# zd87pl/ai-crypto-trader

Hardware: AMD Instinct MI355X
Metric: backtested_1m_candles_per_sec_ga_pop_eval (higher is better)
Workload: dtype fp32; 1 GPU; model=ga_backtest_evolution, global_batch=1024, seq_len=1000000, parallelism=dp1, symbols=64, pop_per_gpu=1024, fitness_segments=64

## Files before the change

ai_crypto_trader_amd/ops/hip/backtest.hip:

```cpp

#include "bt_position.hpp"

namespace {

struct BtState {
    VoteState v;
    BtPosition pos;

    __device__ void load(const float* __restrict__ pr, float initial_equity)
    {
        v.load(pr);
        pos.load(pr, initial_equity);
    }

    __device__ void step(int t, float close, float high, float low,
                         float change, float2 ms, float4 sv)
    {
#pragma clang fp contract(off)
        const int net =
            v.count(t, close, v.recur(t, close, change), ms, sv);
        pos.step(t, net, v.entry_v, v.exit_v, close, high, low);
    }
};

#define BT_BBSUB 32
static_assert(BT_TILE % BT_BBSUB == 0, "sub-tiles must tile the tile");
static_assert(BT_BLOCK % BT_MAXWIN == 0 && BT_BBSUB <= BT_BLOCK &&
                  (BT_MAXWIN & (BT_MAXWIN - 1)) == 0,
              "a lane converts slots of one window only");
static_assert(BT_MAXWIN <= BT_WARMUP, "early-window entries are unused");

__device__ inline float4 bt_pack_sums(double a, double b)
{
    return make_float4(__int_as_float(__double2loint(a)),
                       __int_as_float(__double2hiint(a)),
                       __int_as_float(__double2loint(b)),
                       __int_as_float(__double2hiint(b)));
}

__device__ inline double bt_unpack_sum(float lo, float hi)
{
    return __hiloint2double(__float_as_int(hi), __float_as_int(lo));
}

template <bool HAS_RESNAP>
__global__ void __launch_bounds__(BT_BLOCK, 5) backtest_kernel(
    const float* __restrict__ candles,
    const float* __restrict__ pop,
    float* __restrict__ metrics,
    int nsym, int T, int P, int chunks_per_sym, float initial_equity)
{
#pragma clang fp contract(off)
    __shared__ float chist[BT_SPAN];
    __shared__ double csq[BT_SPAN];
    __shared__ float hl[BT_SPAN][2];
    __shared__ float4 sh_vote[BT_TILE];
    __shared__ float4 bbtab[BT_BBSUB * BT_MAXWIN];
    __shared__ double sh_sum[BT_MAXWIN], sh_sum2[BT_MAXWIN];
    __shared__ double sh_invw[BT_MAXWIN];

    int sym, chunk;
    bt_block_map(blockIdx.x, nsym, chunks_per_sym, sym, chunk);
    const int tid = threadIdx.x;
    const int p = chunk * BT_BLOCK + tid;
    const bool act = p < P;

    BtState st;
    st.load(pop + (long)(act ? p : 0) * BT_NPARAM, initial_equity);
    const float4* my_bb = bbtab + (st.v.bb_w - 2);

    const int scan_w = tid + 2;
    const bool is_scan = scan_w <= BT_MAXWIN;
    if (tid < BT_MAXWIN) {
        BollState b;
        b.init(scan_w);
        sh_sum[tid] = b.sum;
        sh_sum2[tid] = b.sum2;
        sh_invw[tid] = b.inv_w;
    }
    if (tid < BT_BBSUB)
        bbtab[tid * BT_MAXWIN + BT_MAXWIN - 1] =
            make_float4(0.0f, 0.0f, 0.0f, 0.0f);

    float prev_close = 0.f;
    const float4* sym_candles =
        reinterpret_cast<const float4*>(candles + (long)sym * T * 4);

    for (int t0 = 0; t0 < T; t0 += BT_TILE) {
        bt_stage_tile(sym_candles, t0, T, chist, hl, csq);
        const int tend = min(BT_TILE, T - t0);
        const bool resnap_tile = HAS_RESNAP && (t0 > 0) &&
                                 ((t0 & (BT_RESNAP - 1)) == 0);
        if (resnap_tile && is_scan) {
            BollState b;
            b.resnap(scan_w, &chist[BT_HALO]);
            sh_sum[tid] = b.sum;
            sh_sum2[tid] = b.sum2;
        }
        bt_shared_votes(t0, tend, chist, hl, sh_vote);
        for (int s0 = 0; s0 < tend; s0 += BT_BBSUB) {
            const int send = min(s0 + BT_BBSUB, tend);
            if (s0 > 0) __syncthreads();
            if (is_scan) {
                BollState b;
                b.sum = sh_sum[tid];
                b.sum2 = sh_sum2[tid];
#pragma unroll 4
                for (int tt = s0; tt < send; ++tt) {
                    const int i = tt + BT_HALO;
                    if (!(resnap_tile && tt == 0))
                        b.advance(chist[i], chist[i - scan_w], csq[i],
                                  csq[i - scan_w]);
                    bbtab[(tt - s0) * BT_MAXWIN + tid] =
                        bt_pack_sums(b.sum, b.sum2);
                }
                sh_sum[tid] = b.sum;
                sh_sum2[tid] = b.sum2;
            }
            __syncthreads();
            {
                BollState b;
                b.inv_w = sh_invw[tid & (BT_MAXWIN - 1)];
                for (int e = tid; e < (send - s0) * BT_MAXWIN;
                     e += BT_BLOCK) {
                    const float4 v = bbtab[e];
                    b.sum = bt_unpack_sum(v.x, v.y);
                    b.sum2 = bt_unpack_sum(v.z, v.w);
                    const float2 ms = b.stats<false>(0, 0);
                    bbtab[e].x = ms.x;
                    bbtab[e].y = ms.y;
                }
            }
            __syncthreads();
            for (int tt = s0; tt < send; ++tt) {
                const int t = t0 + tt;
                const float close = chist[tt + BT_HALO];
                const float high = hl[tt + BT_HALO][0];
                const float low = hl[tt + BT_HALO][1];
                const float change = (t == 0) ? 0.0f : close - prev_close;
                const float4 sv = sh_vote[tt];
                const float4* e = &my_bb[(tt - s0) * BT_MAXWIN];
                st.step(t, close, high, low, change,
                        make_float2(e->x, e->y), sv);
                prev_close = close;
            }
        }
    }

    if (act)
        st.pos.acc.finalize(metrics + ((long)p * nsym + sym) * BT_NMETRIC, T);
}

}

extern "C" void launch_backtest(const float* candles, const float* pop,
                                float* metrics, int nsym, int T, int P,
                                float initial_equity, hipStream_t stream) {
    const int chunks = (P + BT_BLOCK - 1) / BT_BLOCK;
    auto k = T > BT_RESNAP ? backtest_kernel<true> : backtest_kernel<false>;
    hipLaunchKernelGGL(k, dim3(nsym * chunks), dim3(BT_BLOCK), 0, stream,
                       candles, pop, metrics, nsym, T, P, chunks,
                       initial_equity);
}
```

ai_crypto_trader_amd/ops/hip/bt_common.hpp:

```cpp
#pragma once

#include "common.hpp"

#define BT_BLOCK 256
#define BT_TILE 256
#define BT_NMETRIC 10
#define BT_FEE 0.001f
#define BT_EPS 1e-9f
#define BT_ANNUALIZE 0x1.6a7dccp+9f

__device__ inline void bt_write_metrics(
    float* __restrict__ out, int T, float equity, float n_trades,
    float wins, float gross_p, float gross_l, float max_dd, float sum_ret,
    float sum_ret2)
{
#pragma clang fp contract(off)
    float n = (float)max(T, 1);
    float mean_r = sum_ret / n;
    float var_r = fmaxf(sum_ret2 / n - mean_r * mean_r, 0.0f);
    float sharpe = mean_r / fmaxf(sqrtf(var_r), BT_EPS) * BT_ANNUALIZE;
    if (!(n_trades > 0.0f)) sharpe = 0.0f;
    float win_rate = wins / fmaxf(n_trades, 1.0f);
    float fitness = (n_trades > 0.0f)
                        ? sharpe + win_rate - 2.0f * max_dd
                        : -1.0f;
    out[0] = equity; out[1] = n_trades; out[2] = wins;
    out[3] = gross_p; out[4] = gross_l; out[5] = max_dd;
    out[6] = sum_ret; out[7] = sum_ret2;
    out[8] = sharpe; out[9] = fitness;
}

struct BtAccum {
    float equity, max_eq, max_dd;
    float n_trades, wins, gross_p, gross_l;
    float sum_ret, sum_ret2;

    __device__ void init(float initial_equity)
    {
        equity = initial_equity; max_eq = initial_equity; max_dd = 0.f;
        n_trades = wins = gross_p = gross_l = 0.f;
        sum_ret = sum_ret2 = 0.f;
    }

    __device__ void trade(float pnl)
    {
        n_trades += 1.0f;
        wins += (pnl > 0.0f) ? 1.0f : 0.0f;
        gross_p += fmaxf(pnl, 0.0f);
        gross_l += fmaxf(-pnl, 0.0f);
    }

    __device__ void mark(float new_eq)
    {
#pragma clang fp contract(off)
        float r = new_eq / equity - 1.0f;
        sum_ret += r;
        sum_ret2 += r * r;
        equity = new_eq;
        max_eq = fmaxf(max_eq, equity);
        max_dd = fmaxf(max_dd, (max_eq - equity) / max_eq);
    }

    __device__ void finalize(float* __restrict__ out, int T) const
    {
        bt_write_metrics(out, T, equity, n_trades, wins, gross_p, gross_l,
                         max_dd, sum_ret, sum_ret2);
    }
};

__device__ inline void bt_block_map(int bid, int nsym, int chunks_per_sym,
                                    int& sym, int& chunk)
{
    int nblocks = nsym * chunks_per_sym;
    if ((nsym & 7) == 0 && (nblocks & 7) == 0) {
        int xcd = bid & 7, j = bid >> 3;
        sym = xcd + 8 * (j / chunks_per_sym);
        chunk = j % chunks_per_sym;
    } else {
        sym = bid / chunks_per_sym;
        chunk = bid % chunks_per_sym;
    }
}
```

ai_crypto_trader_amd/ops/hip/bt_position.hpp:

```cpp
#pragma once

#include "bt_vote.hpp"

#define BT_EV_NONE 0
#define BT_EV_STOP 1
#define BT_EV_TP 2
#define BT_EV_SIGNAL 3
#define BT_EV_ENTRY (-1)

struct BtEvent {
    int kind;
    float price;
    float pnl;
};

struct BtPosition {
    float size_pct, sl_pct, tp_pct, trail_pct, trail_act;
    float cash, units;
    bool in_pos;
    float entry_cost, entry_price;
    float stop, tp, peak;
    BtAccum acc;

    __device__ void load(const float* __restrict__ pr, float initial_equity)
    {
        size_pct = pr[12]; sl_pct = pr[13]; tp_pct = pr[14];
        trail_pct = pr[15]; trail_act = pr[16];
        cash = initial_equity; units = 0.f;
        in_pos = false;
        entry_cost = entry_price = stop = tp = peak = 0.f;
        acc.init(initial_equity);
    }

    __device__ BtEvent step(int t, int net, int entry_v, int exit_v,
                            float close, float high, float low)
    {
#pragma clang fp contract(off)
        BtEvent ev = {BT_EV_NONE, 0.0f, 0.0f};
        if (in_pos) {
            peak = fmaxf(peak, high);
            bool trail_on = (trail_pct > 0.0f) &&
                            (peak >= entry_price * (1.0f + trail_act));
            if (trail_on)
                stop = fmaxf(stop, peak * (1.0f - trail_pct));
            bool hit_sl = low <= stop;
            bool hit_tp = !hit_sl && high >= tp;
            bool hit_sig = !hit_sl && !hit_tp && net <= -exit_v;
            if (hit_sl || hit_tp || hit_sig) {
                float exit_price = hit_sl ? stop : (hit_tp ? tp : close);
                float proceeds = units * exit_price * (1.0f - BT_FEE);
                cash += proceeds;
                acc.trade(proceeds - entry_cost);
                ev.kind = hit_sl ? BT_EV_STOP
                                 : (hit_tp ? BT_EV_TP : BT_EV_SIGNAL);
                ev.price = exit_price;
                ev.pnl = proceeds - entry_cost;
                units = 0.0f;
                in_pos = false;
            }
        } else if (t >= BT_WARMUP && net >= entry_v) {
            float cost = fminf(size_pct * acc.equity, cash);
            units = cost * (1.0f - BT_FEE) / close;
            cash -= cost;
            entry_cost = cost;
            entry_price = close;
            stop = close * (1.0f - sl_pct);
            tp = close * (1.0f + tp_pct);
            peak = close;
            in_pos = true;
            ev.kind = BT_EV_ENTRY;
        }

        if (units != 0.0f || cash != acc.equity)
            acc.mark(cash + units * close);
        return ev;
    }
};
```

ai_crypto_trader_amd/ops/hip/bt_vote.hpp:

```cpp
#pragma once

#include "bt_common.hpp"

#define BT_NPARAM 19
#define BT_MAXWIN 32
#define BT_HALO 64
#define BT_SPAN (BT_TILE + BT_HALO)
#define BT_WARMUP 128
#define BT_RESNAP 16384
#define BT_NSTATE 18

struct BollState {
    double sum, sum2, inv_w;

    __device__ void init(int w)
    {
        sum = sum2 = 0.0;
        inv_w = 1.0 / (double)w;
    }

    __device__ void resnap(int w, const float* __restrict__ hist)
    {
#pragma clang fp contract(off)
        double s = 0.0, s2 = 0.0;
        for (int j = BT_MAXWIN - 1; j >= 0; --j) {
            if (j < w) {
                double c = (double)hist[-j];
                s += c;
                s2 += c * c;
            }
        }
        sum = s;
        sum2 = s2;
    }

    __device__ void advance(float close, float oldc, double csq_new,
                            double csq_old)
    {
#pragma clang fp contract(off)
        double old = (double)oldc;
        double c64 = (double)close;
        sum += c64 - old;
        sum2 += csq_new - csq_old;
    }

    template <bool EARLY = true>
    __device__ float2 stats(int t, int w) const
    {
#pragma clang fp contract(off)
        double inv_cnt = inv_w;
        if (EARLY && t < BT_MAXWIN && t + 1 < w)
            inv_cnt = 1.0 / (t + 1.0);
        double mean64 = sum * inv_cnt;
        double var64 = fmax(sum2 * inv_cnt - mean64 * mean64, 0.0);
        return make_float2((float)mean64, sqrtf((float)var64));
    }
};

struct VoteState {
    float inv_rsi_p, rsi_os, rsi_ob;
    float a_f, a_s, a_sig;
    int bb_w;
    float bb_k, bb_bth, bb_sth;
    int entry_v, exit_v;
    float stoch_os, stoch_ob, will_os, will_ob;

    float ema_f, ema_s, sig;
    float avg_gain, avg_loss;
    BollState bb;

    __device__ void load(const float* __restrict__ pr)
    {
        inv_rsi_p = 1.0f / fmaxf(floorf(pr[0]), 1.0f);
        rsi_os = pr[1]; rsi_ob = pr[2];
        a_f = 2.0f / (pr[3] + 1.0f);
        a_s = 2.0f / (pr[4] + 1.0f);
        a_sig = 2.0f / (pr[5] + 1.0f);
        bb_w = min(max((int)pr[6], 2), BT_MAXWIN);
        bb_k = pr[7]; bb_bth = pr[8]; bb_sth = pr[9];
        entry_v = (int)pr[10]; exit_v = (int)pr[11];
        stoch_os = pr[17]; stoch_ob = pr[18];
        will_os = stoch_os - 100.0f;
        will_ob = stoch_ob - 100.0f;
        ema_f = ema_s = sig = 0.f;
        avg_gain = avg_loss = 0.f;
        bb.init(bb_w);
    }

    __device__ void resnap(const float* __restrict__ hist)
    {
        bb.resnap(bb_w, hist);
    }

    __device__ void warm_step(float close, float change)
    {
#pragma clang fp contract(off)
        ema_f += a_f * (close - ema_f);
        ema_s += a_s * (close - ema_s);
        float macd = ema_f - ema_s;
        sig += a_sig * (macd - sig);
        float gain = fmaxf(change, 0.0f);
        float loss = fmaxf(-change, 0.0f);
        avg_gain += (gain - avg_gain) * inv_rsi_p;
        avg_loss += (loss - avg_loss) * inv_rsi_p;
    }

    struct Osc { float macd_hist, rsi_num, rsi_den; };

    __device__ Osc recur(int t, float close, float change)
    {
#pragma clang fp contract(off)
        if (t == 0) { ema_f = close; ema_s = close; }
        else {
            ema_f += a_f * (close - ema_f);
            ema_s += a_s * (close - ema_s);
        }
        float macd = ema_f - ema_s;
        sig += a_sig * (macd - sig);
        Osc o;
        o.macd_hist = macd - sig;

        float gain = fmaxf(change, 0.0f);
        float loss = fmaxf(-change, 0.0f);
        avg_gain += (gain - avg_gain) * inv_rsi_p;
        avg_loss += (loss - avg_loss) * inv_rsi_p;
        o.rsi_num = 100.0f * avg_gain;
        o.rsi_den = avg_gain + fmaxf(avg_loss, BT_EPS);
        return o;
    }

    __device__ int count(int t, float close, Osc o, float2 ms,
                         float4 sv) const
    {
#pragma clang fp contract(off)
        float band = bb_k * ms.y;
        float bb_num = close - (ms.x - band);
        float bb_den = fmaxf(2.0f * band, BT_EPS);

        int net = 0;
        if (t >= BT_WARMUP) {
            int buy = (o.rsi_num < rsi_os * o.rsi_den) +
                      (o.macd_hist > 0.0f) +
                      (bb_num < bb_bth * bb_den) +
                      (sv.x < stoch_os * sv.z) +
                      (sv.y < will_os * sv.z);
            int sell = (o.rsi_num > rsi_ob * o.rsi_den) +
                       (o.macd_hist < 0.0f) +
                       (bb_num > bb_sth * bb_den) +
                       (sv.x > stoch_ob * sv.z) +
                       (sv.y > will_ob * sv.z);
            net = buy - sell + __float_as_int(sv.w);
        }
        return net;
    }

    template <bool SKIP_BB>
    __device__ int step(int t, float close, float change, float oldc,
                        double csq_new, double csq_old, float4 sv)
    {
        const Osc o = recur(t, close, change);
        if (!SKIP_BB) bb.advance(close, oldc, csq_new, csq_old);
        return count(t, close, o, bb.stats(t, bb_w), sv);
    }
};

__device__ inline void bt_stage_tile(
    const float4* __restrict__ sym_candles, int t0, int T,
    float* __restrict__ chist, float (*__restrict__ hl)[2],
    double* __restrict__ csq)
{
#pragma clang fp contract(off)
    __syncthreads();
    for (int i = threadIdx.x; i < BT_SPAN; i += BT_BLOCK) {
        const int t = t0 - BT_HALO + i;
        float4 c = make_float4(0.0f, 0.0f, 0.0f, 0.0f);
        if (t >= 0 && t < T) c = sym_candles[t];
        chist[i] = c.x;
        if (csq) csq[i] = (double)c.x * (double)c.x;
        hl[i][0] = c.y;
        hl[i][1] = c.z;
    }
    __syncthreads();
}

__device__ inline void bt_shared_votes(
    int t0, int tend, const float* __restrict__ chist,
    const float (*__restrict__ hl)[2], float4* __restrict__ sh_vote)
{
#pragma clang fp contract(off)
    const int tid = threadIdx.x;
    if (tid >= tend) return;
    const int t = t0 + tid;
    const int base = tid + BT_HALO;
    const float cl = chist[base];
    const int L14 = min(t + 1, 14);
    float hmax = -1e30f, lmin = 1e30f;
    for (int j = 0; j < L14; ++j) {
        hmax = fmaxf(hmax, hl[base - j][0]);
        lmin = fminf(lmin, hl[base - j][1]);
    }
    const int L20 = min(t + 1, 20);
    double s20 = 0.0;
    for (int j = 0; j < L20; ++j) s20 += (double)chist[base - j];
    const float sma20 = (float)(s20 / (double)L20);
    const int L50 = min(t + 1, 50);
    double s50 = 0.0;
    for (int j = 0; j < L50; ++j) s50 += (double)chist[base - j];
    const float sma50 = (float)(s50 / (double)L50);
    const int trend = (cl > sma20 && sma20 > sma50) ? 1
                      : ((cl < sma20 && sma20 < sma50) ? -1 : 0);
    sh_vote[tid] = make_float4(
        100.0f * (cl - lmin), -100.0f * (hmax - cl),
        fmaxf(hmax - lmin, BT_EPS), __int_as_float(trend));
}
```

Baseline: 412.5 billion candles/s.

## Precompute per-step candle records, skip warm-up vote work, trim register pressure

Thread blocks now write a per-timestep record (close, high, low, change) next to the vote data in shared memory, so the serial loop does one float4 load instead of several scalar loads and no longer carries prev_close. Warm-up sub-tiles only advance the oscillator recurrences and skip Bollinger stat conversion and the vote/position logic, which also removes the t>=WARMUP tests from the main path. Trailing-stop multipliers are precomputed at load, and inline asm v_max/v_min plus asm volatile barriers on tid keep values in VGPRs and reduce live registers. This raises shared memory use and relies on hand-written asm that may block compiler scheduling.

```diff
diff --git a/ai_crypto_trader_amd/ops/hip/backtest.hip b/ai_crypto_trader_amd/ops/hip/backtest.hip
--- a/ai_crypto_trader_amd/ops/hip/backtest.hip
+++ b/ai_crypto_trader_amd/ops/hip/backtest.hip
@@ -11,20 +11,27 @@
     {
         v.load(pr);
         pos.load(pr, initial_equity);
+        asm volatile("" : "+v"(v.will_os), "+v"(v.will_ob));
     }
 
-    __device__ void step(int t, float close, float high, float low,
-                         float change, float2 ms, float4 sv)
+    __device__ void step(int t, float4 c, float2 ms, float4 sv)
     {
 #pragma clang fp contract(off)
-        const int net =
-            v.count(t, close, v.recur(t, close, change), ms, sv);
-        pos.step(t, net, v.entry_v, v.exit_v, close, high, low);
+        const int net = v.count<false>(
+            t, c.x, v.recur<true>(t, c.x, c.w), ms, sv);
+        pos.step<false>(t, net, v.entry_v, v.exit_v, c.x, c.y, c.z);
+    }
+
+    __device__ void warm(int t, float4 c)
+    {
+        v.recur<true>(t, c.x, c.w);
     }
 };
 
 #define BT_BBSUB 32
 static_assert(BT_TILE % BT_BBSUB == 0, "sub-tiles must tile the tile");
+static_assert(BT_WARMUP % BT_BBSUB == 0 && BT_WARMUP <= BT_TILE,
+              "the warm-up is whole sub-tiles of the first tile");
 static_assert(BT_BLOCK % BT_MAXWIN == 0 && BT_BBSUB <= BT_BLOCK &&
                   (BT_MAXWIN & (BT_MAXWIN - 1)) == 0,
               "a lane converts slots of one window only");
@@ -54,7 +61,7 @@
     __shared__ float chist[BT_SPAN];
     __shared__ double csq[BT_SPAN];
     __shared__ float hl[BT_SPAN][2];
-    __shared__ float4 sh_vote[BT_TILE];
+    __shared__ float4 rec[BT_TILE][2];
     __shared__ float4 bbtab[BT_BBSUB * BT_MAXWIN];
     __shared__ double sh_sum[BT_MAXWIN], sh_sum2[BT_MAXWIN];
     __shared__ double sh_invw[BT_MAXWIN];
@@ -69,11 +76,9 @@
     st.load(pop + (long)(act ? p : 0) * BT_NPARAM, initial_equity);
     const float4* my_bb = bbtab + (st.v.bb_w - 2);
 
-    const int scan_w = tid + 2;
-    const bool is_scan = scan_w <= BT_MAXWIN;
     if (tid < BT_MAXWIN) {
         BollState b;
-        b.init(scan_w);
+        b.init(tid + 2);
         sh_sum[tid] = b.sum;
         sh_sum2[tid] = b.sum2;
         sh_invw[tid] = b.inv_w;
@@ -82,46 +87,56 @@
         bbtab[tid * BT_MAXWIN + BT_MAXWIN - 1] =
             make_float4(0.0f, 0.0f, 0.0f, 0.0f);
 
-    float prev_close = 0.f;
     const float4* sym_candles =
         reinterpret_cast<const float4*>(candles + (long)sym * T * 4);
+    if (T > 0) st.v.ema_f = st.v.ema_s = sym_candles[0].x;
 
     for (int t0 = 0; t0 < T; t0 += BT_TILE) {
-        bt_stage_tile(sym_candles, t0, T, chist, hl, csq);
+        int ltid = tid;
+        asm volatile("" : "+v"(ltid));
+        const int scan_w = ltid + 2;
+        const bool is_scan = scan_w <= BT_MAXWIN;
+        bt_stage_tile(sym_candles, t0, T, chist, hl, csq, ltid);
         const int tend = min(BT_TILE, T - t0);
         const bool resnap_tile = HAS_RESNAP && (t0 > 0) &&
                                  ((t0 & (BT_RESNAP - 1)) == 0);
         if (resnap_tile && is_scan) {
             BollState b;
             b.resnap(scan_w, &chist[BT_HALO]);
-            sh_sum[tid] = b.sum;
-            sh_sum2[tid] = b.sum2;
+            sh_sum[ltid] = b.sum;
+            sh_sum2[ltid] = b.sum2;
         }
-        bt_shared_votes(t0, tend, chist, hl, sh_vote);
+        bt_shared_votes<true>(t0, tend, chist, hl, &rec[0][0], ltid);
         for (int s0 = 0; s0 < tend; s0 += BT_BBSUB) {
             const int send = min(s0 + BT_BBSUB, tend);
+            const bool warm = t0 + s0 < BT_WARMUP;
             if (s0 > 0) __syncthreads();
             if (is_scan) {
                 BollState b;
-                b.sum = sh_sum[tid];
-                b.sum2 = sh_sum2[tid];
+                b.sum = sh_sum[ltid];
+                b.sum2 = sh_sum2[ltid];
 #pragma unroll 4
                 for (int tt = s0; tt < send; ++tt) {
                     const int i = tt + BT_HALO;
                     if (!(resnap_tile && tt == 0))
                         b.advance(chist[i], chist[i - scan_w], csq[i],
                                   csq[i - scan_w]);
-                    bbtab[(tt - s0) * BT_MAXWIN + tid] =
+                    bbtab[(tt - s0) * BT_MAXWIN + ltid] =
                         bt_pack_sums(b.sum, b.sum2);
                 }
-                sh_sum[tid] = b.sum;
-                sh_sum2[tid] = b.sum2;
+                sh_sum[ltid] = b.sum;
+                sh_sum2[ltid] = b.sum2;
             }
             __syncthreads();
+            if (warm) {
+                for (int tt = s0; tt < send; ++tt)
+                    st.warm(t0 + tt, rec[tt][0]);
+                continue;
+            }
             {
                 BollState b;
-                b.inv_w = sh_invw[tid & (BT_MAXWIN - 1)];
-                for (int e = tid; e < (send - s0) * BT_MAXWIN;
+                b.inv_w = sh_invw[ltid & (BT_MAXWIN - 1)];
+                for (int e = ltid; e < (send - s0) * BT_MAXWIN;
                      e += BT_BLOCK) {
                     const float4 v = bbtab[e];
                     b.sum = bt_unpack_sum(v.x, v.y);
@@ -133,22 +148,19 @@
             }
             __syncthreads();
             for (int tt = s0; tt < send; ++tt) {
-                const int t = t0 + tt;
-                const float close = chist[tt + BT_HALO];
-                const float high = hl[tt + BT_HALO][0];
-                const float low = hl[tt + BT_HALO][1];
-                const float change = (t == 0) ? 0.0f : close - prev_close;
-                const float4 sv = sh_vote[tt];
                 const float4* e = &my_bb[(tt - s0) * BT_MAXWIN];
-                st.step(t, close, high, low, change,
-                        make_float2(e->x, e->y), sv);
-                prev_close = close;
+                st.step(t0 + tt, rec[tt][0], make_float2(e->x, e->y),
+                        rec[tt][1]);
             }
         }
     }
 
-    if (act)
-        st.pos.acc.finalize(metrics + ((long)p * nsym + sym) * BT_NMETRIC, T);
+    int otid = tid;
+    asm volatile("" : "+v"(otid));
+    const int po = chunk * BT_BLOCK + otid;
+    if (po < P)
+        st.pos.acc.finalize(metrics + ((long)po * nsym + sym) * BT_NMETRIC,
+                            T);
 }
 
 }
diff --git a/ai_crypto_trader_amd/ops/hip/bt_common.hpp b/ai_crypto_trader_amd/ops/hip/bt_common.hpp
--- a/ai_crypto_trader_amd/ops/hip/bt_common.hpp
+++ b/ai_crypto_trader_amd/ops/hip/bt_common.hpp
@@ -8,6 +8,41 @@
 #define BT_FEE 0.001f
 #define BT_EPS 1e-9f
 #define BT_ANNUALIZE 0x1.6a7dccp+9f
+
+__device__ __forceinline__ float bt_max(float a, float b)
+{
+    float r;
+    asm("v_max_f32 %0, %1, %2" : "=v"(r) : "v"(a), "v"(b));
+    return r;
+}
+
+__device__ __forceinline__ float bt_min(float a, float b)
+{
+    float r;
+    asm("v_min_f32 %0, %1, %2" : "=v"(r) : "v"(a), "v"(b));
+    return r;
+}
+
+__device__ __forceinline__ float bt_max_uniform(float uniform, float b)
+{
+    float r;
+    asm("v_max_f32 %0, %1, %2" : "=v"(r) : "s"(uniform), "v"(b));
+    return r;
+}
+
+__device__ __forceinline__ float bt_pos_part(float x)
+{
+    float r;
+    asm("v_max_f32 %0, 0, %1" : "=v"(r) : "v"(x));
+    return r;
+}
+
+__device__ __forceinline__ float bt_neg_part(float x)
+{
+    float r;
+    asm("v_max_f32 %0, -%1, 0" : "=v"(r) : "v"(x));
+    return r;
+}
 
 __device__ inline void bt_write_metrics(
     float* __restrict__ out, int T, float equity, float n_trades,
@@ -57,8 +92,8 @@
         sum_ret += r;
         sum_ret2 += r * r;
         equity = new_eq;
-        max_eq = fmaxf(max_eq, equity);
-        max_dd = fmaxf(max_dd, (max_eq - equity) / max_eq);
+        max_eq = bt_max(max_eq, equity);
+        max_dd = bt_max(max_dd, (max_eq - equity) / max_eq);
     }
 
     __device__ void finalize(float* __restrict__ out, int T) const
diff --git a/ai_crypto_trader_amd/ops/hip/bt_position.hpp b/ai_crypto_trader_amd/ops/hip/bt_position.hpp
--- a/ai_crypto_trader_amd/ops/hip/bt_position.hpp
+++ b/ai_crypto_trader_amd/ops/hip/bt_position.hpp
@@ -15,34 +15,39 @@
 };
 
 struct BtPosition {
-    float size_pct, sl_pct, tp_pct, trail_pct, trail_act;
+    float size_pct, sl_pct, tp_pct;
+    float trail_m, act_m;
+    bool trail_en;
     float cash, units;
     bool in_pos;
     float entry_cost, entry_price;
+    float trail_trig;
     float stop, tp, peak;
     BtAccum acc;
 
     __device__ void load(const float* __restrict__ pr, float initial_equity)
     {
+#pragma clang fp contract(off)
         size_pct = pr[12]; sl_pct = pr[13]; tp_pct = pr[14];
-        trail_pct = pr[15]; trail_act = pr[16];
+        trail_m = 1.0f - pr[15]; act_m = 1.0f + pr[16];
+        trail_en = pr[15] > 0.0f;
         cash = initial_equity; units = 0.f;
         in_pos = false;
-        entry_cost = entry_price = stop = tp = peak = 0.f;
+        entry_cost = entry_price = trail_trig = stop = tp = peak = 0.f;
         acc.init(initial_equity);
     }
 
+    template <bool WARM_TEST = true>
     __device__ BtEvent step(int t, int net, int entry_v, int exit_v,
                             float close, float high, float low)
     {
 #pragma clang fp contract(off)
         BtEvent ev = {BT_EV_NONE, 0.0f, 0.0f};
         if (in_pos) {
-            peak = fmaxf(peak, high);
-            bool trail_on = (trail_pct > 0.0f) &&
-                            (peak >= entry_price * (1.0f + trail_act));
+            peak = bt_max(peak, high);
+            bool trail_on = trail_en && (peak >= trail_trig);
             if (trail_on)
-                stop = fmaxf(stop, peak * (1.0f - trail_pct));
+                stop = bt_max(stop, peak * trail_m);
             bool hit_sl = low <= stop;
             bool hit_tp = !hit_sl && high >= tp;
             bool hit_sig = !hit_sl && !hit_tp && net <= -exit_v;
@@ -58,12 +63,13 @@
                 units = 0.0f;
                 in_pos = false;
             }
-        } else if (t >= BT_WARMUP && net >= entry_v) {
-            float cost = fminf(size_pct * acc.equity, cash);
+        } else if ((!WARM_TEST || t >= BT_WARMUP) && net >= entry_v) {
+            float cost = bt_min(size_pct * acc.equity, cash);
             units = cost * (1.0f - BT_FEE) / close;
             cash -= cost;
             entry_cost = cost;
             entry_price = close;
+            trail_trig = close * act_m;
             stop = close * (1.0f - sl_pct);
             tp = close * (1.0f + tp_pct);
             peak = close;
diff --git a/ai_crypto_trader_amd/ops/hip/bt_vote.hpp b/ai_crypto_trader_amd/ops/hip/bt_vote.hpp
--- a/ai_crypto_trader_amd/ops/hip/bt_vote.hpp
+++ b/ai_crypto_trader_amd/ops/hip/bt_vote.hpp
@@ -107,10 +107,11 @@
 
     struct Osc { float macd_hist, rsi_num, rsi_den; };
 
+    template <bool SEEDED = false>
     __device__ Osc recur(int t, float close, float change)
     {
 #pragma clang fp contract(off)
-        if (t == 0) { ema_f = close; ema_s = close; }
+        if (!SEEDED && t == 0) { ema_f = close; ema_s = close; }
         else {
             ema_f += a_f * (close - ema_f);
             ema_s += a_s * (close - ema_s);
@@ -120,15 +121,17 @@
         Osc o;
         o.macd_hist = macd - sig;
 
-        float gain = fmaxf(change, 0.0f);
-        float loss = fmaxf(-change, 0.0f);
+        float gain = SEEDED ? bt_pos_part(change) : fmaxf(change, 0.0f);
+        float loss = SEEDED ? bt_neg_part(change) : fmaxf(-change, 0.0f);
         avg_gain += (gain - avg_gain) * inv_rsi_p;
         avg_loss += (loss - avg_loss) * inv_rsi_p;
         o.rsi_num = 100.0f * avg_gain;
-        o.rsi_den = avg_gain + fmaxf(avg_loss, BT_EPS);
+        o.rsi_den = avg_gain + (SEEDED ? bt_max_uniform(BT_EPS, avg_loss)
+                                       : fmaxf(avg_loss, BT_EPS));
         return o;
     }
 
+    template <bool WARM_TEST = true>
     __device__ int count(int t, float close, Osc o, float2 ms,
                          float4 sv) const
     {
@@ -138,7 +141,7 @@
         float bb_den = fmaxf(2.0f * band, BT_EPS);
 
         int net = 0;
-        if (t >= BT_WARMUP) {
+        if (!WARM_TEST || t >= BT_WARMUP) {
             int buy = (o.rsi_num < rsi_os * o.rsi_den) +
                       (o.macd_hist > 0.0f) +
                       (bb_num < bb_bth * bb_den) +
@@ -167,11 +170,11 @@
 __device__ inline void bt_stage_tile(
     const float4* __restrict__ sym_candles, int t0, int T,
     float* __restrict__ chist, float (*__restrict__ hl)[2],
-    double* __restrict__ csq)
+    double* __restrict__ csq, int tid = threadIdx.x)
 {
 #pragma clang fp contract(off)
     __syncthreads();
-    for (int i = threadIdx.x; i < BT_SPAN; i += BT_BLOCK) {
+    for (int i = tid; i < BT_SPAN; i += BT_BLOCK) {
         const int t = t0 - BT_HALO + i;
         float4 c = make_float4(0.0f, 0.0f, 0.0f, 0.0f);
         if (t >= 0 && t < T) c = sym_candles[t];
@@ -183,12 +186,13 @@
     __syncthreads();
 }
 
+template <bool RECORD = false>
 __device__ inline void bt_shared_votes(
     int t0, int tend, const float* __restrict__ chist,
-    const float (*__restrict__ hl)[2], float4* __restrict__ sh_vote)
+    const float (*__restrict__ hl)[2], float4* __restrict__ sh_vote,
+    int tid = threadIdx.x)
 {
 #pragma clang fp contract(off)
-    const int tid = threadIdx.x;
     if (tid >= tend) return;
     const int t = t0 + tid;
     const int base = tid + BT_HALO;
@@ -209,7 +213,11 @@
     const float sma50 = (float)(s50 / (double)L50);
     const int trend = (cl > sma20 && sma20 > sma50) ? 1
                       : ((cl < sma20 && sma20 < sma50) ? -1 : 0);
-    sh_vote[tid] = make_float4(
+    if (RECORD)
+        sh_vote[2 * tid] = make_float4(
+            cl, hl[base][0], hl[base][1],
+            (t == 0) ? 0.0f : cl - chist[base - 1]);
+    sh_vote[RECORD ? 2 * tid + 1 : tid] = make_float4(
         100.0f * (cl - lmin), -100.0f * (hmax - cl),
         fmaxf(hmax - lmin, BT_EPS), __int_as_float(trend));
 }
```

New measurement: 439.4 billion candles/s (median of 6 runs). +6.5%, better.
